# So-bonkers/Detecting-Convolutional-Codes-Via-Markovian-Statistics

Hardware: AMD Instinct MI355X
Metric: MC trials/sec at N=1e5, rate-1/2 m=6 pair, 1/2/4/8 GPUs; Pd match vs CPU (higher is better)
Workload: dtype u32 bit-planes (metrics, four planes of the 64 states) + f64 (log-likelihood sums)

## Files before the change

### detecting-convolutional-codes-via-markovian-statistics_amd/csrc/cvd_device.h

```cpp
#pragma once
#ifndef __HIPCC_RTC__
#include <hip/hip_runtime.h>
#include <stdint.h>
#include <stddef.h>
#else
typedef unsigned char uint8_t;
typedef int int32_t;
typedef unsigned int uint32_t;
typedef long long int64_t;
typedef unsigned long long uint64_t;
typedef __SIZE_TYPE__ size_t;
#endif
#include "cvd_keys.h"
#include "cvd_bitslice.h"

namespace cvd_dev {

using cvd::kEmptyKey;
using cvd::row_words_c;
using cvd::key_hash;

constexpr int kBlock = 256;
#ifndef CVD_K1B_LDSF
#define CVD_K1B_LDSF 0
// ... 60 lines not shown
  if ((threadIdx.x & 63) == 0) {
    if (b1) atomicAdd(reinterpret_cast<unsigned long long*>(counts), (unsigned long long)__popcll(b1));
    if (b2) atomicAdd(reinterpret_cast<unsigned long long*>(counts + 1), (unsigned long long)__popcll(b2));
  }
}

__device__ __forceinline__ int early_decide(double lp, double lr, int64_t rem, double lt_min, double lp_min) {
  const double f = 1.0 + (double)(4 * rem + 32) * 0x1p-53;
  if (lp <= (lr + (double)rem * lt_min) * f) return 1;
  if ((lp + (double)rem * lp_min) * f > lr) return 2;
  return 0;
}
__device__ __forceinline__ void early_final(int dec, double& lp, double& lr) {
  if (dec == 1) { lp = -1.0; lr = 0.0; }
  if (dec == 2) { lp = 1.0; lr = 0.0; }
}
constexpr int kEarlyEvery = 128;


struct ExpArgs {
  const uint32_t* filt;
  const uint32_t* hkey;
  const uint32_t* hrow;
  const uint32_t* drow;
  const uint32_t* dkey;
  const uint32_t* t2;
  const double* ltref;
  const uint32_t* bmp;
  uint32_t repmap, swmap;
  uint32_t bfly_uni;
  uint32_t bfly_even[4];
  uint32_t hmask, fmask, fmask4;
  uint32_t ksh, rsh;
  int32_t max_probe;
  int32_t slot0;
  double lp_unseen;
  int64_t N, nseq, n_h1;
  const uint32_t* r;
  double* sums;
  int64_t* counts;
  uint8_t* trace;
  int32_t early;
  int32_t walk;
  int32_t walk_wmin, walk_amin, walk_burst;
  double lt_min, lp_min;
  int32_t* err;
  const uint32_t* pf;
  uint32_t* wq;
  int32_t mix;
  int32_t t2c;
  int32_t nvtab;
  uint32_t vtab_off;
  const double* vtab;
  int32_t ck_n;
  int32_t ck_len, ck_warm;
  uint32_t* ck_out;
};
constexpr int kCkRecWords = 20;

template <int n>
struct StreamReader {
  static constexpr int SPW = 32 / n;
  static constexpr uint32_t MASK = (1u << n) - 1u;
  const uint32_t* r;
  int64_t pitch, q, N, nwords, wi;
  uint4 cache;
// ... 781 lines not shown
```

### detecting-convolutional-codes-via-markovian-statistics_amd/csrc/cvd_host.cpp

```cpp
#include <atomic>
#include <chrono>
#include <functional>
#include <map>
#include <mutex>
#include <thread>
#include <tuple>
#include <cstdlib>
#include <exception>
#include <cstdio>
#include <algorithm>
#include <cmath>
#include <cstring>
#include <memory>
#include <new>
#include <stdexcept>
#include <string>
#include <unordered_map>
#include <vector>

#include <sys/stat.h>
#include <unistd.h>

#include "../../include/cvd.h"
#include "cvd_internal.h"
// ... 486 lines not shown
    Mo.h_key_slot[(size_t)i] = (uint32_t)slot;
    slot_of[(size_t)i] = (int64_t)slot;
  }
  pt.mark("  nibble tables: hash + insert");
  Mo.h_dkey.assign((size_t)Mo.n_rows * nw, 0u);
  const Tabs T = make_tabs(Mo.dec);
  parallel_for(Mo.n_rows, [&](int64_t i, int) {
    uint32_t* dw = Mo.h_drow.data() + (size_t)dev_of[(size_t)i] * Mo.h_rsw;
    const uint8_t* D = Mo.keys.data() + (size_t)i * M;
    uint8_t succ[16][256];
    for (int r = 0; r < R; ++r) step_host(T, D, (uint32_t)r, succ[r]);
    for (int r = 0; r < R; ++r) {
      std::memcpy(dw + 4 * r, Mo.logp1.data() + (size_t)i * R + r, sizeof(double));
      const int64_t j = Mo.row_next[(size_t)i * R + r];
      dw[4 * r + 2] = (uint32_t)(j >= 0 ? (int32_t)dev_of[(size_t)j] : -1);
      uint32_t c = 0u;
      for (int q2 = 0; q2 < R; ++q2) c += std::memcmp(succ[q2], succ[r], (size_t)M) == 0;
      dw[4 * r + 3] = c;
    }
    std::memcpy(Mo.h_dkey.data() + (size_t)dev_of[(size_t)i] * nw, kws.data() + (size_t)i * nw,
                sizeof(uint32_t) * (size_t)nw);
    uint32_t* hw = interleave ? Mo.h_key_rows.data() + (size_t)i * ssw + nw
                              : Mo.h_row_rows.data() + (size_t)i * Mo.h_rsw;
    std::memcpy(hw, dw, sizeof(uint32_t) * Mo.h_rsw);
  });
  Mo.slot0 = (int32_t)dev_of[0];
  pt.mark("  nibble tables: records");
  Mo.bs = bitslice_preferred(Mo);
  int bload = 3;
  if (const char* e = std::getenv("CVD_BS_LOAD_LOG2")) bload = std::max(1, std::min(5, std::atoi(e)));
  int64_t bcap = 64;
  while (bcap < ((int64_t)1 << bload) * Mo.n_rows) bcap <<= 1;
  constexpr int kSlotW = 64;
  if (bcap * 4 * kSlotW > ((int64_t)1 << 32) || Mo.n_rows * 512 > ((int64_t)1 << 32)) Mo.bs = false;
  Mo.h_bfilt.clear(); Mo.h_bfilt_lds.clear(); Mo.h_bkey_rows.clear(); Mo.h_bkey_slot.clear(); Mo.h_bdkey.clear();
  Mo.h_bpf.clear();
  Mo.bhcap = 0; Mo.bmax_probe = 0;
  if (Mo.bs) {
    Mo.bs_pat_bits = kFilterPatBits;
    if (const char* e = std::getenv("CVD_BS_PAT_BITS")) Mo.bs_pat_bits = std::max(8, std::min(kFilterPatBits, std::atoi(e)));
    const bool bpf = bs_pf_preferred(Mo, ldsf);
    if (bpf) {
      Mo.bs_pat_bits = std::min(Mo.bs_pat_bits, (int32_t)kFilterPatBitsLds);
      Mo.bs_pf_log2 = kBsPfLog2Bits;
      if (const char* e = std::getenv("CVD_BS_PF_LOG2")) Mo.bs_pf_log2 = std::max(16, std::min(20, std::atoi(e)));
      Mo.h_bpf.assign((size_t)1 << (Mo.bs_pf_log2 - 5), 0u);
    }
    const unsigned bnpat = 1u << Mo.bs_pat_bits;
    Mo.bhcap = bcap;
    constexpr int kRecW = 48, kImgW = 48;
    Mo.h_bkey_rows.assign((size_t)Mo.n_rows * kSlotW, 0u);
    Mo.h_bkey_slot.assign((size_t)Mo.n_rows, 0u);
    Mo.h_bfilt.assign((size_t)fcap, 0u);
    Mo.h_bfilt_lds.assign(ldsf ? (size_t)fcap : 0u, 0u);
    Mo.h_bdkey.assign((size_t)Mo.n_rows * kImgW, 0u);
    pt.mark("  bit-sliced tables: allocate");
    std::vector<uint32_t> bph((size_t)Mo.n_rows), bpl((size_t)Mo.n_rows);
    parallel_for(Mo.n_rows, [&](int64_t i, int) {
      uint32_t z[2];
      bs_digest(Mo.keys.data() + (size_t)i * M, z);
      bs_key_hash(z[0], z[1], bph[(size_t)i], bpl[(size_t)i]);
    });
    std::vector<uint8_t> used((size_t)bcap, 0);
    for (int64_t i = 0; i < Mo.n_rows; ++i) {
      const uint32_t ph = bph[(size_t)i], pl = bpl[(size_t)i];
      const size_t fb = (size_t)filter_block_index(pl, (uint32_t)(fcap / 2 - 1));
      Mo.h_bfilt[2 * fb] |= filter_pattern(filter_pattern_index(ph, bnpat));
// ... 632 lines not shown
```

### detecting-convolutional-codes-via-markovian-statistics_amd/csrc/cvd_k1s.h

```cpp
#pragma once

#if defined(CVD_K1S_SLOT3) || defined(CVD_K1S_DEEP) || defined(CVD_K1S_T2) || defined(CVD_K1S_TRIM) || \
    defined(CVD_K1S_MIDPOS) || defined(CVD_K1S_VMASK) || defined(CVD_K1S_PADV) || defined(CVD_K1S_ABL) || \
    defined(CVD_WALK_BUF) || defined(CVD_K1S_AMASK) || defined(CVD_K1S_R16) || defined(CVD_K1S_NT_STREAM) || \
    defined(CVD_BS_ETAB2)
#error "removed k1s knob: CVD_K1S_SLOT3, CVD_K1S_DEEP, CVD_K1S_T2, CVD_K1S_TRIM, CVD_K1S_MIDPOS, CVD_K1S_VMASK, CVD_K1S_PADV, CVD_K1S_ABL, CVD_WALK_BUF, CVD_K1S_AMASK, CVD_K1S_R16, CVD_K1S_NT_STREAM and CVD_BS_ETAB2 no longer exist (DESIGN.md §10)"
#endif

#ifndef CVD_K1B_BITSLICE
#define CVD_K1B_BITSLICE 0
#endif

namespace cvd_dev {

constexpr int kBsSlotShift = 6;
constexpr int kBsRecWord = 48;
template <int PH>
__device__ __forceinline__ constexpr uint32_t bs_img_off() { return 32u * PH; }
constexpr uint32_t kBsRecOff = 4u * kBsRecWord;
constexpr int kBsDkeyWords = 48;
constexpr int kBsEarlyGroups = 21;
#ifndef CVD_K1S_PF
#define CVD_K1S_PF 0
#endif
// ... 43 lines not shown
  }
}
template <int PH, bool kUni, class Mid>
__device__ __forceinline__ void bs_core_tab(const uint32_t (&R)[2][4], uint32_t rr, uint32_t (&N)[2][4], uint32_t& c,
                                            bool& one, Mid mid) {
  const uint2 E0 = *reinterpret_cast<const uint2*>(reinterpret_cast<const char*>(bs_e0_lds()) + PH * 64 + rr);
  const uint32_t e0[2] = {E0.x, E0.y};
  uint32_t mu;
  cvd::bs_step_core_tab<PH, kUni>(
      R, e0,
      [&](bool zero_hit) {
        const char* tb = reinterpret_cast<const char*>(bs_mt_lds()) + PH * 128;
        const uint32_t o = rr + (zero_hit ? 0u : 64u);
        const uint4 w0 = *reinterpret_cast<const uint4*>(tb + o);
        const uint4 w1 = *reinterpret_cast<const uint4*>(tb + o + kBsMtSub);
        const uint2 q = *reinterpret_cast<const uint2*>(tb + o + 2u * kBsMtSub);
        cvd::BsMu T;
        T.e0m[0] = w0.x; T.a1[0] = w0.y; T.p1[0] = w0.z; T.a23[0] = w0.w;
        T.e0m[1] = w1.x; T.a1[1] = w1.y; T.p1[1] = w1.z; T.a23[1] = w1.w;
        T.p23[0] = q.x; T.p23[1] = q.y;
        return T;
      },
      N, mu, c, mid, &one);
}
__device__ __forceinline__ void bs_lt_add(double& lr, const double* s_lt, double lt1, uint32_t c, bool one) {
  if (__builtin_expect(one, 1)) {
    lr += lt1;
  } else {
    lr += s_lt[c];
    asm volatile("" : "+v"(lr));
  }
}

struct BsCursor {
  int32_t slot, pnx;
  uint32_t hs, hsn, fb, fw, fb1, fw1, pc;
  bool cand;
  bool pfpos = true;
  bool h2wave = false;
  double plp;
  uint32_t pkey[8];
  uint32_t vhmask = 0u, vfmask4 = 0u;
  uint32_t half;
  __device__ void prefetch_row(const ExpArgs& a, int32_t s, uint32_t rn) {
    uint32_t o;
    asm("v_lshl_add_u32 %0, %1, 6, %2" : "=v"(o) : "v"((uint32_t)s), "v"(rn));
    const uint4 v = ld_off<uint4>(a.drow, o);
    pc = v.w;
    pnx = (int32_t)v.z;
    plp = __hiloint2double((int)v.y, (int)v.x);
  }
  __device__ void start(const ExpArgs& a, uint32_t r0) {
    slot = a.slot0; hs = 0u; hsn = 0u; fb = 0u; fw = 0u; fb1 = 0u; fw1 = 0u; cand = false; pc = 1u; half = 0u;
    prefetch_row(a, slot, r0);
  }
  __device__ void fence_mid(uint32_t dep) {
    asm volatile("" : "+v"(fw), "+v"(fw1), "+v"(slot) : "v"(dep));
  }
  __device__ void fence_resolve(uint32_t dep) {
    asm volatile("" : "+v"(slot), "+v"(pnx), "+v"(plp), "+v"(pc) : "v"(dep));
#pragma unroll
    for (int w = 0; w < 8; ++w) asm volatile("" : "+v"(pkey[w]) : "v"(dep));
  }
  __device__ static uint32_t slot_off(uint32_t s) { return s << (kBsSlotShift + 2); }
  __device__ static void load_image(const uint32_t* base, uint32_t o, uint32_t (&k)[8]) {
    const uint4 u = ld_off<uint4>(base, o), v = ld_off<uint4>(base, o + 16u);
    k[0] = u.x; k[1] = u.y; k[2] = u.z; k[3] = u.w; k[4] = v.x; k[5] = v.y; k[6] = v.z; k[7] = v.w;
  }
  template <int PH>
  __device__ void mid(const ExpArgs& a, uint32_t r) {
    cand = slot == -2 && cvd::bs_bop3<cvd::kTtAndNotOr>(fb1, fw1, cvd::bs_bop3<cvd::kTtAndNotOr>(fb, fw, 0u)) == 0u;
    if (cand) {
      const uint32_t so = slot_off(hs);
      load_image(a.hkey, so + bs_img_off<PH>(), pkey);
      const uint4 v = ld_off<uint4>(a.hkey, so + kBsRecOff + r);
      pc = v.w;
      pnx = (int32_t)v.z;
      plp = __hiloint2double((int)v.y, (int)v.x);
    }
  }
  __device__ static bool same(const uint32_t (&k)[8], const uint32_t (&R)[2][4]) {
    uint32_t d = k[0] ^ R[0][0];
    d = cvd::bs_bop3<cvd::kTtXorOr>(k[1], R[0][1], d);
    d = cvd::bs_bop3<cvd::kTtXorOr>(k[2], R[0][2], d);
    d = cvd::bs_bop3<cvd::kTtXorOr>(k[3], R[0][3], d);
    d = cvd::bs_bop3<cvd::kTtXorOr>(k[4], R[1][0], d);
    d = cvd::bs_bop3<cvd::kTtXorOr>(k[5], R[1][1], d);
    d = cvd::bs_bop3<cvd::kTtXorOr>(k[6], R[1][2], d);
    d = cvd::bs_bop3<cvd::kTtXorOr>(k[7], R[1][3], d);
    asm volatile("" : "+v"(d));
    return d == 0u;
  }
  template <int PH>
  __device__ double resolve(const ExpArgs& a, const uint32_t (&R)[2][4], uint32_t r, double lpu) {
    const uint32_t m = (uint32_t)(slot >> 31);
    double lpv = lpu;
    int32_t ns = -2;
    ns = (int32_t)cvd::bs_bop3<cvd::kTtSel>(m, (uint32_t)-2, (uint32_t)pnx);
    lpv =
        __hiloint2double((int)cvd::bs_bop3<cvd::kTtSel>(m, (uint32_t)__double2hiint(lpu), (uint32_t)__double2hiint(plp)),
                         (int)cvd::bs_bop3<cvd::kTtSel>(m, (uint32_t)__double2loint(lpu), (uint32_t)__double2loint(plp)));
    if (cand) {
      if (same(pkey, R)) {
        lpv = plp; ns = pnx;
      } else if (pc != 0u) {
        uint32_t sl = hs;
        for (int pr = 1; pr <= a.max_probe; ++pr) {
          sl = (sl + 1u) & a.hmask;
          const uint32_t so = slot_off(sl);
          const uint4 v = ld_off<uint4>(a.hkey, so + kBsRecOff + r);
          if (v.w == 0u) break;
          uint32_t k[8];
          load_image(a.hkey, so + bs_img_off<PH>(), k);
          if (same(k, R)) {
            lpv = __hiloint2double((int)v.y, (int)v.x);
            ns = (int32_t)v.z;
            break;
          }
        }
      }
    }
    slot = ns;
    half = 0u;
    return lpv;
  }
  template <int PH>
  __device__ void hash_ahead(const ExpArgs& a, const uint32_t (&N)[2][4]) {
    uint32_t ph, pl;
    cvd::bs_digest_hash<PH>(N, ph, pl);
    hsn = ph & a.hmask;
    const uint2 pp = *reinterpret_cast<const uint2*>(reinterpret_cast<const char*>(filter_patterns_lds()) +
                                                     (ph & (uint32_t)((cvd::kFilterPatterns - 1) << 3)));
    fb = pp.x;
    fb1 = pp.y;
#if CVD_K1S_PF
    const uint32_t pfw = reinterpret_cast<const uint32_t*>(dyn_lds())[__builtin_amdgcn_ubfe(
        pl, 32 - cvd::kBsPfLog2Bits + 5, cvd::kBsPfLog2Bits - 5)];
    const uint32_t pbit = __builtin_amdgcn_ubfe(pfw, pl >> (32 - cvd::kBsPfLog2Bits), 1u);
    const uint32_t pm = 0u - pbit, sm = (uint32_t)(slot >> 31);
    fb = cvd::bs_bop3<0xF3>(fb, pm, 0u);
    fb1 = cvd::bs_bop3<0xF3>(fb1, pm, 0u);
    const uint32_t fo = cvd::bs_bop3<0x80>(pl, pm, sm) & a.fmask4;
#else
    const uint32_t fo = slot < 0 ? (pl & a.fmask4) : 0u;
#endif
#if CVD_K1B_LDSF
    const uint2 f = *reinterpret_cast<const uint2*>(reinterpret_cast<const char*>(dyn_lds()) + fo);
#else
    const uint2 f = ld_off<uint2>(a.filt, fo);
#endif
    fw = f.x;
    fw1 = f.y;
  }
  template <bool kRow = true>
  __device__ void next(const ExpArgs& a, uint32_t rn) {
    if (kRow && slot >= 0) prefetch_row(a, slot, rn);
    hs = hsn;
  }
};

template <int PH, bool kUni>
__device__ __forceinline__ void bs_step(const ExpArgs& a, BsCursor& cur, const uint32_t (&R)[2][4], uint32_t rr,
                                        uint32_t (&N)[2][4], uint32_t& c, bool& one) {
  bs_core_tab<PH, kUni>(R, rr, N, c, one, [&](uint32_t dep) {
    cur.fence_mid(dep);
    cur.template mid<PH>(a, rr);
  });
  cur.template hash_ahead<(PH + 1) % 6>(a, N);
  cur.fence_resolve(N[1][3]);
}

template <uint64_t XM>
__device__ __forceinline__ void k1s_walk(const ExpArgs& a, int64_t qwave, uint64_t vmask, const double* s_lt) {
  constexpr bool kUni = xm_uni<6, XM>();
  if (CVD_WALK_ABL & 1) return;
  const bool valid = qwave + lane_id() < a.nseq;
  const uint32_t N = (uint32_t)a.N;
  const uint32_t nwords = (N + 15u) / 16u;
  const size_t cstride = (size_t)a.nseq * 4;
  auto load_word = [&](uint32_t wi) -> uint32_t {
    if (wi >= nwords) return 0u;
    return a.r[(size_t)(wi >> 2) * cstride + (size_t)(qwave + lane_id()) * 4 + (wi & 3u)];
  };
  uint32_t pos = 0u, curw = 0u, nxtw = 0u;
  bool need = false;
  auto cur_word = [&]() -> uint32_t { return curw; };
  auto nxt_word = [&]() -> uint32_t { return nxtw; };
  auto word_at = [&]() -> uint32_t { return cur_word() >> (2u * (pos & 15u)); };
  auto advance = [&]() {
    ++pos;
    if ((pos & 15u) == 0u) {
      curw = nxtw;
      need = true;
    }
  };
  uint32_t R[2][4] = {{0u, 0u, 0u, 0u}, {0u, 0u, 0u, 0u}};
  double lp = 0.0, lr = 0.0;
  BsCursor cur;
  cur.slot = -1; cur.pnx = -1; cur.hs = 0u; cur.hsn = 0u; cur.fb = 0u; cur.fw = 0u; cur.fb1 = 0u; cur.fw1 = 0u;
// ... 15 lines not shown
      uint32_t o;
      asm("v_lshl_add_u32 %0, %1, 5, %2" : "=v"(o) : "v"(x & 15u), "v"((uint32_t)cur.slot << 9));
      const uint4 v = ld_off<uint4>(a.t2, o);
      const uint2 w = ld_off<uint2>(a.t2, o + 16u);
      cur.pc = w.y;
      cur.pnx = (int32_t)w.x;
      plp2 = __hiloint2double((int)v.w, (int)v.z);
      cur.plp = __hiloint2double((int)v.y, (int)v.x);
    } else {
      cur.prefetch_row(a, cur.slot, word_param(x & 3u));
    }
  };
  uint32_t mode = kWalkDone;
  int dec = 0;
  auto finished = [&]() -> bool {
    if (pos == N) return true;
    if (a.early && (pos & (uint32_t)(kEarlyEvery - 1)) == 0u) dec = early_decide(lp, lr, (int64_t)(N - pos), a.lt_min, a.lp_min);
    return dec != 0;
  };
  if (valid && N > 0u) {
    curw = load_word(0u);
    nxtw = load_word(1u);
    cur.slot = a.slot0;
    walk_prefetch();
    mode = kWalkWalk;
  }
  uint32_t phw = 0u;
  const double lt1 = a.ltref[1];
  auto acs_step = [&](auto phc) {
    constexpr int PH = decltype(phc)::value;
    const uint32_t rr = word_param(word_at() & 3u);
    uint32_t Nn[2][4], c;
    bool one;
    bs_step<PH, kUni>(a, cur, R, rr, Nn, c, one);
    if (mode == kWalkAcs) {
      lp += cur.template resolve<PH>(a, R, rr, a.lp_unseen);
      bs_lt_add(lr, s_lt, lt1, c, one);
      advance();
      cur.template next<false>(a, 0u);
      if (finished()) {
        mode = kWalkDone;
        cur.slot = -1;
      } else if (cur.slot >= 0) {
        mode = kWalkWalk;
        walk_prefetch();
      }
    }
#pragma unroll
    for (int r = 0; r < 2; ++r)
#pragma unroll
      for (int i = 0; i < 4; ++i) R[r][i] = Nn[r][i];
  };
  const uint32_t wmin = (uint32_t)a.walk_wmin, amin = (uint32_t)a.walk_amin;
  const int burst = a.walk_burst;
  for (int64_t it = 0, it_max = CVD_WALK_GUARD * ((int64_t)N + 1); it < it_max; ++it) {
    if (need) {
      nxtw = load_word((pos >> 4) + 1u);
      need = false;
    }
    const uint64_t mA = __ballot(mode == kWalkAcs), mW = __ballot(mode == kWalkWalk);
    if ((mA | mW) == 0u) break;
    const uint32_t nA = (uint32_t)__popcll(mA), nW = (uint32_t)__popcll(mW);
    if (nW != 0u && (nA == 0u || nW >= wmin || nA < amin)) {
      for (int b = 0; b < burst; ++b) {
        if (mode == kWalkWalk) {
          auto leave = [&]() {
            if (CVD_WALK_ABL & 8) {
              cur.slot = a.slot0;
              advance();
              if (finished()) {
                mode = kWalkDone;
                cur.slot = -1;
// ... 104 lines not shown
  }
  if ((CVD_WALK_ABL & 4) && a.walk) return;
  double lp = 0.0, lr = 0.0;
  if (valid) {
    uint32_t R[2][4] = {{0u, 0u, 0u, 0u}, {0u, 0u, 0u, 0u}};
    double lpu = a.lp_unseen;
    asm volatile("" : "+v"(lpu));
    const int64_t N = a.N, nwords = (N + 15) / 16;
    const size_t cstride = (size_t)a.nseq * 4;
    constexpr bool ck = kCk;
    int64_t t_begin = 0, t_sum = 0, t_end = N;
    if (ck) {
      t_sum = (int64_t)ck_j * a.ck_len;
      t_end = min(N, t_sum + (int64_t)a.ck_len);
      t_begin = max((int64_t)0, t_sum - (int64_t)a.ck_warm);
    }
    uint32_t c4[4];
    auto load_chunk = [&](int64_t ci) {
      const uint32_t* rb = a.r + (size_t)ci * cstride + (size_t)qwave * 4;
      const uint4 v = 4 * ci < nwords ? stream_load(reinterpret_cast<const uint4*>(rb + lane_id() * 4u))
                                      : make_uint4(0u, 0u, 0u, 0u);
      c4[0] = v.x; c4[1] = v.y; c4[2] = v.z; c4[3] = v.w;
    };
    auto pick = [&](int64_t wi) -> uint32_t {
      const uint32_t e = (uint32_t)wi & 3u;
      const uint32_t v = e == 0u ? c4[0] : e == 1u ? c4[1] : e == 2u ? c4[2] : c4[3];
      return wi < nwords ? v : 0u;
    };
    int64_t wi = t_begin / 16;
    load_chunk(wi >> 2);
    uint32_t cw = pick(wi), nw = pick(wi + 1);
    uint32_t sh = 0u;
    BsCursor cur;
    cur.start(a, word_param(cw & 3u));
    const double lt1 = a.ltref[1];
    auto step = [&](auto phc, uint32_t rr, uint32_t rn) {
      constexpr int PH = decltype(phc)::value;
      uint32_t Nn[2][4], c;
      bool one;
      bs_step<PH, kUni>(a, cur, R, rr, Nn, c, one);
      lp += cur.template resolve<PH>(a, R, rr, lpu);
      bs_lt_add(lr, s_lt, lt1, c, one);
#pragma unroll
      for (int r = 0; r < 2; ++r)
#pragma unroll
        for (int i = 0; i < 4; ++i) R[r][i] = Nn[r][i];
      cur.next(a, rn);
    };
    int64_t t = t_begin;
    int grp = 0, dec = 0;
    auto wk = [&](uint32_t w5, auto kc) -> uint32_t {
      constexpr uint32_t k = decltype(kc)::value;
      return (w5 >> (k + 1)) & 0x30u;
    };
    for (; t + 6 <= t_end; t += 6) {
      if (ck && t == t_sum) {
        ck_store(a, qwave, ck_j, 0u, R);
        lp = 0.0;
        lr = 0.0;
      }
      const uint32_t win = __builtin_amdgcn_alignbit(nw, cw, sh);
      const uint32_t w5 = win << 5;
      step(IntC<0>{}, wk(w5, IntC<0>{}), wk(w5, IntC<2>{}));
      step(IntC<1>{}, wk(w5, IntC<2>{}), wk(w5, IntC<4>{}));
      step(IntC<2>{}, wk(w5, IntC<4>{}), wk(w5, IntC<6>{}));
      step(IntC<3>{}, wk(w5, IntC<6>{}), wk(w5, IntC<8>{}));
      step(IntC<4>{}, wk(w5, IntC<8>{}), wk(w5, IntC<10>{}));
      step(IntC<5>{}, wk(w5, IntC<10>{}), wk(w5, IntC<12>{}));
      sh += 12u;
      if (sh >= 32u) {
        sh -= 32u;
        ++wi;
        cw = nw;
        nw = pick(wi + 1);
        if (((wi + 1) & 3) == 3) load_chunk((wi + 2) >> 2);
      }
      if (a.early && ++grp == kBsEarlyGroups) {
        grp = 0;
        if (!dec) dec = early_decide(lp, lr, N - (t + 6), a.lt_min, a.lp_min);
        if (__ballot(dec == 0) == 0) {
          t = N;
          break;
        }
      }
    }
    const int ntail = (int)(t_end - t);
    (void)ntail;
    if (t < t_end) {
      if (ck && t == t_sum) {
        ck_store(a, qwave, ck_j, 0u, R);
        lp = 0.0;
        lr = 0.0;
      }
      const uint32_t win = __builtin_amdgcn_alignbit(nw, cw, sh);
      const uint32_t w5 = win << 5;
      step(IntC<0>{}, wk(w5, IntC<0>{}), wk(w5, IntC<2>{}));
      if (t + 1 < t_end) step(IntC<1>{}, wk(w5, IntC<2>{}), wk(w5, IntC<4>{}));
      if (t + 2 < t_end) step(IntC<2>{}, wk(w5, IntC<4>{}), wk(w5, IntC<6>{}));
      if (t + 3 < t_end) step(IntC<3>{}, wk(w5, IntC<6>{}), wk(w5, IntC<8>{}));
      if (t + 4 < t_end) step(IntC<4>{}, wk(w5, IntC<8>{}), wk(w5, IntC<10>{}));
    }
    if (ck) {
      ck_store(a, qwave, ck_j, 8u, R);
      uint32_t l = lane_id();
      asm volatile("" : "+v"(l));
      double* ps = reinterpret_cast<double*>(
          a.ck_out + ((size_t)ck_j * (size_t)a.nseq + (size_t)qwave + l) * kCkRecWords + 16u);
      ps[0] = lp;
      ps[1] = lr;
      return;
    }
    if (a.sums) {
      const int64_t qe = qwave + lane_id();
      a.sums[2 * qe] = lp;
      a.sums[2 * qe + 1] = lr;
    }
    early_final(dec, lp, lr);
  }
  if constexpr (kCk) return;
  count_decisions_masked(vmask, hmask, lp, lr, a.counts);
// ... 66 lines not shown
```

### detecting-convolutional-codes-via-markovian-statistics_amd/csrc/cvd_kernels.hip

```cpp
#include <hip/hip_runtime.h>

#include <algorithm>
#include <atomic>
#include <cstdlib>
#include <cstring>
#include <map>
#include <mutex>
#include <string>

#include "../../include/cvd.h"
#include "cvd_common.h"
#include "cvd_internal.h"
#include "cvd_device.h"

using namespace cvd;

#define HIP_CHECK(x)                                                                      \
  do {                                                                                    \
    hipError_t e_ = (x);                                                                  \
    if (e_ != hipSuccess) {                                                               \
      set_error(std::string("HIP error '") + hipGetErrorString(e_) + "' at " #x);          \
      return CVD_E_HIP;                                                                   \
    }                                                                                     \
  } while (0)
// ... 1240 lines not shown
}

ExpKernel pick_explicit(int m, int k, int n) {
  if (k == 1 && n == 2) {
    switch (m) {
      case 2: return detect_explicit_kernel<2, 1, 2>;
      case 3: return detect_explicit_kernel<3, 1, 2>;
      case 4: return detect_explicit_kernel<4, 1, 2>;
      case 5: return detect_explicit_kernel<5, 1, 2>;
      case 6: return detect_explicit_kernel<6, 1, 2>;
    }
  }
  if (m == 4 && k == 2 && n == 3) return detect_explicit_kernel<4, 2, 3>;
  return nullptr;
}

template <typename T>
int dev_copy(T*& d, const std::vector<T>& h) {
  if (h.empty()) return CVD_OK;
  HIP_CHECK(hipMalloc(&d, h.size() * sizeof(T)));
  HIP_CHECK(hipMemcpy(d, h.data(), h.size() * sizeof(T), hipMemcpyHostToDevice));
  return CVD_OK;
}

__global__ __launch_bounds__(kBlock) void dir_scatter_kernel(const uint32_t* rows, const uint32_t* slots, int64_t n,
                                                             int32_t w, uint32_t* dir) {
  const int64_t idx = (int64_t)blockIdx.x * kBlock + threadIdx.x;
  if (idx >= n * w) return;
  const int64_t i = idx / w, k = idx - i * w;
  dir[(size_t)slots[i] * (size_t)w + (size_t)k] = rows[idx];
}

int dev_directory(uint32_t*& d, const std::vector<uint32_t>& rows, const std::vector<uint32_t>& slots, int64_t cap,
                  int32_t w, uint32_t fill) {
  if (rows.empty() || cap <= 0) return CVD_OK;
  const int64_t n = (int64_t)slots.size();
  if ((int64_t)rows.size() != n * w) { set_error("directory rows / slots mismatch"); return CVD_E_INVALID; }
  HIP_CHECK(hipMalloc(&d, (size_t)cap * (size_t)w * sizeof(uint32_t)));
  HIP_CHECK(hipMemsetD32(d, (int)fill, (size_t)cap * (size_t)w));
  uint32_t *dr = nullptr, *ds = nullptr;
  HIP_CHECK(hipMalloc(&dr, rows.size() * sizeof(uint32_t)));
  HIP_CHECK(hipMalloc(&ds, slots.size() * sizeof(uint32_t)));
  HIP_CHECK(hipMemcpy(dr, rows.data(), rows.size() * sizeof(uint32_t), hipMemcpyHostToDevice));
  HIP_CHECK(hipMemcpy(ds, slots.data(), slots.size() * sizeof(uint32_t), hipMemcpyHostToDevice));
  const unsigned grid = (unsigned)((n * w + kBlock - 1) / kBlock);
  hipLaunchKernelGGL(dir_scatter_kernel, dim3(grid), dim3(kBlock), 0, 0, dr, ds, n, w, d);
  HIP_CHECK(hipGetLastError());
  HIP_CHECK(hipDeviceSynchronize());
  HIP_CHECK(hipFree(dr));
  HIP_CHECK(hipFree(ds));
  return CVD_OK;
}

}


int cvd::check_device(const cvd_model& M) {
  if (M.device < 0) { set_error("model not uploaded (cvd_model_upload)"); return CVD_E_STATE; }
  int cur = -1;
  HIP_CHECK(hipGetDevice(&cur));
  if (cur != M.device) { set_error("current device differs from the model's device"); return CVD_E_INVALID; }
  return CVD_OK;
}

namespace {
GenArgs gen_args(const CodeDesc& enc, uint32_t k0, uint32_t k1, uint32_t tag, uint64_t thr, int64_t N,
                 int random_input) {
  GenArgs a;
  a.enc = enc; a.k0 = k0; a.k1 = k1; a.tag = tag;
  a.thr_all = thr >= (1ull << 32); a.thr_lo = (uint32_t)std::min<uint64_t>(thr, 0xFFFFFFFFull);
  a.random_input = random_input; a.N = N;
  a.seq_base = 0; a.seq_stride = 1; a.pitch = 0; a.q0 = 0; a.count = 0; a.r = nullptr;
// ... 299 lines not shown
  const bool bs = M.rtc_fn ? M.rtc_bs : bitslice_preferred(M);
  return walk_preferred(M) || (env_i("CVD_LDSF_LOCKSTEP", bs ? 1 : 0) == 1);
}
bool cvd::ldsf_preferred(const cvd_model& M) {
  return !std::getenv("CVD_NO_LDSF") && ldsf_wanted(M) && M.n_rows <= ldsf_max_rows(M.bs) &&
         M.fcap <= ((int64_t)1 << ldsf_log2(M.bs)) && M.h_filt_lds.size() == (size_t)M.fcap;
}

bool cvd::walk_preferred(const cvd_model& M, bool early) {
  const int e = env_i("CVD_WALK", -1);
  if (e >= 0) return e != 0;
  if (M.rtc_fn ? M.rtc_bs : bitslice_preferred(M)) return false;
  return !early && M.kind == 1 && M.learn_len_eff > 0 && 10 * M.n_rows < M.learn_len_eff;
}

static int64_t persist_cap(const cvd_model& M) {
  if (!M.rtc_fn || !M.rtc_bs || M.rtc_persist_grid <= 0 || env_i("CVD_K1S_PERSIST", 1) == 0) return 0;
  int64_t g = M.rtc_persist_grid;
  if (const int pb = env_i("CVD_K1S_PERSIST_BLOCKS", 0); pb > 0) g = std::min<int64_t>(g, pb);
  return g;
}
int64_t cvd::persist_seqs(const cvd_model& M) { return persist_cap(M) * M.rtc_block; }
int64_t cvd::persist_grid(const cvd_model& M, int64_t nseq) {
  const int64_t g = persist_cap(M);
  return g > 0 && (nseq + M.rtc_block - 1) / M.rtc_block > g ? g : 0;
}

static unsigned rtc_dyn_lds(const cvd_model& M) {
  if (M.rtc_ldsf) return (unsigned)(M.fcap * sizeof(uint32_t) + (M.rtc_t2c ? M.h_vtab.size() * sizeof(double) : 0));
  if (M.rtc_pf) return (unsigned)(M.h_bpf.size() * sizeof(uint32_t));
  return 0u;
}

static ExpArgs exp_args(const cvd_model& M, int which, const uint32_t* d_r, int64_t N, int64_t nseq, int64_t n_h1,
                        double* d_sums, int64_t* d_counts, uint8_t* d_trace, const uint32_t* bmp, bool early) {
  ExpArgs a;
  const bool bs = which == CVD_KERNEL_BUTTERFLY_RTC && M.rtc_bs;
  a.filt = which == CVD_KERNEL_BUTTERFLY_RTC && M.rtc_ldsf ? (bs ? M.d_bfilt_lds : M.d_filt_lds)
                                                            : (bs ? M.d_bfilt : M.d_filt);
  a.hkey = bs ? M.d_bkey : M.d_hkey; a.drow = M.d_drow; a.ltref = M.d_ltref;
  a.hrow = bs ? M.d_bkey : M.d_hrow ? M.d_hrow : M.d_hkey + nib_words(M.dec.m);
  a.ksh = bs ? 8u : (uint32_t)__builtin_ctz((unsigned)(4 * M.h_ssw));
  a.rsh = bs ? 8u : M.d_hrow ? (uint32_t)__builtin_ctz((unsigned)(4 * M.h_rsw)) : a.ksh;
  a.bmp = bmp; a.slot0 = M.slot0;
  a.repmap = M.repmap; a.swmap = M.swmap; a.bfly_uni = M.bfly_uni;
  for (int w = 0; w < 4; ++w) a.bfly_even[w] = M.bfly_even[w];
  a.hmask = (uint32_t)((bs ? M.bhcap : M.hcap) - 1); a.fmask = (uint32_t)(M.fcap / 2 - 1); a.fmask4 = a.fmask << 3;
  a.max_probe = bs ? M.bmax_probe : M.max_probe; a.lp_unseen = M.logp1_unseen;
  a.N = N; a.nseq = nseq; a.n_h1 = n_h1; a.r = d_r; a.sums = d_sums; a.counts = d_counts;
  a.trace = d_trace;
  a.early = early && !d_sums && !d_trace; a.lt_min = M.ltref[1]; a.lp_min = M.lp_min;
  a.dkey = bs ? M.d_bdkey : M.d_dkey;
  a.err = M.d_err;
  a.pf = bs && M.rtc_pf ? M.d_bpf : nullptr;
  a.wq = nullptr;
  a.ck_n = 0; a.ck_len = 0; a.ck_warm = 0; a.ck_out = nullptr;
  {
    const int e = env_i("CVD_K1S_MIX", -1);
    a.mix = e >= 0 ? (e != 0) : (M.kind == 1 && M.learn_len_eff > 0 && 2 * M.n_rows < M.learn_len_eff);
  }
  a.t2 = (!M.h_t2.empty() && !std::getenv("CVD_WALK_NOT2")) ? M.d_t2 : nullptr;
  a.t2c = 0; a.nvtab = 0; a.vtab_off = 0u; a.vtab = nullptr;
  if (a.t2 && which == CVD_KERNEL_BUTTERFLY_RTC && M.rtc_bs && M.rtc_ldsf && M.rtc_t2c) {
    a.t2 = M.d_t2c;
    a.t2c = 1;
    a.vtab = M.d_vtab;
    a.nvtab = (int32_t)M.h_vtab.size();
    a.vtab_off = (uint32_t)(M.fcap * sizeof(uint32_t));
  }
  a.walk = which == CVD_KERNEL_BUTTERFLY_RTC && !d_trace && N < ((int64_t)1 << 31) && M.d_dkey && walk_preferred(M, a.early);
  a.walk_wmin = env_i("CVD_WALK_WMIN", 48);
  a.walk_amin = env_i("CVD_WALK_AMIN", 4);
  a.walk_burst = a.t2 ? std::max(1, std::min(7, env_i("CVD_WALK_BURST", 7)))
                      : std::max(1, std::min(16, env_i("CVD_WALK_BURST", 16)));
// ... 249 lines not shown
    for (int32_t c : v) tot += c;
  cvd::ck_last[3] = tot;
  return rc;
}

std::string cvd::rtc_variant_defs(int block, bool ldsf, int patbits, bool bs, bool pf, int pf_log2) {
  return "-DCVD_K1B_BLOCK=" + std::to_string(block) + (ldsf ? " -DCVD_K1B_LDSF=1" : "") +
         (patbits != kFilterPatBits ? " -DCVD_FILTER_PAT_BITS=" + std::to_string(patbits) : "") +
         (bs ? " -DCVD_K1B_BITSLICE=1" : "") + (pf ? " -DCVD_K1S_PF=1" : "") +
         (pf && pf_log2 != kBsPfLog2Bits ? " -DCVD_K1S_PF_LOG2=" + std::to_string(pf_log2) : "");
}

int cvd::upload_model(cvd_model& M, int device) {
  if (M.device == device) return CVD_OK;
  if (M.device >= 0) free_model_device(M);
  int cur = 0;
  HIP_CHECK(hipGetDevice(&cur));
  struct Restore {
    int d;
    ~Restore() { (void)hipSetDevice(d); }
  } restore{cur};
  HIP_CHECK(hipSetDevice(device));
  int rc;
  if ((rc = dev_copy(M.d_ltref, M.ltref))) return rc;
  if (M.kind == 0) {
    if ((rc = dev_copy(M.d_rec, M.rec))) return rc;
    if ((rc = dev_copy(M.d_logp1, M.logp1))) return rc;
  }
  if (M.hcap > 0) {
    if ((rc = dev_copy(M.d_filt, M.h_filt))) return rc;
    if ((rc = dev_copy(M.d_filt_lds, M.h_filt_lds))) return rc;
    if ((rc = dev_directory(M.d_hkey, M.h_key_rows, M.h_key_slot, M.hcap, M.h_ssw, kEmptyKey))) return rc;
    if ((rc = dev_directory(M.d_hrow, M.h_row_rows, M.h_key_slot, M.hcap, M.h_rsw, 0u))) return rc;
    if ((rc = dev_copy(M.d_drow, M.h_drow))) return rc;
    if ((rc = dev_copy(M.d_dkey, M.h_dkey))) return rc;
    if ((rc = dev_copy(M.d_t2, M.h_t2))) return rc;
    if ((rc = dev_copy(M.d_t2c, M.h_t2c))) return rc;
    if ((rc = dev_copy(M.d_vtab, M.h_vtab))) return rc;
    if ((rc = dev_copy(M.d_bfilt, M.h_bfilt))) return rc;
    if ((rc = dev_copy(M.d_bfilt_lds, M.h_bfilt_lds))) return rc;
    if ((rc = dev_directory(M.d_bkey, M.h_bkey_rows, M.h_bkey_slot, M.bhcap, 1 << cvd_dev::kBsSlotShift, 0u))) return rc;
    if ((rc = dev_copy(M.d_bdkey, M.h_bdkey))) return rc;
    if ((rc = dev_copy(M.d_bpf, M.h_bpf))) return rc;
    if ((rc = dev_copy(M.d_bmp, M.bmp))) return rc;
    if ((rc = dev_copy(M.d_bmk1, M.bmk1))) return rc;
    if ((rc = dev_copy(M.d_bfly, M.bfly))) return rc;
  }
  HIP_CHECK(hipMalloc((void**)&M.d_err, sizeof(int32_t)));
  HIP_CHECK(hipMemset(M.d_err, 0, sizeof(int32_t)));
  M.device = device;
  M.lp_min = M.kind == 1 ? M.logp1_unseen : 0.0;
  for (double v : M.logp1) M.lp_min = std::min(M.lp_min, v);
  M.rtc_fn = nullptr;
  M.rtc_fn_multi = nullptr;
  M.rtc_fn_walk = nullptr;
  M.rtc_fn_multi_walk = nullptr;
  M.rtc_nowalk = false;
  M.jit_error.clear();
  M.rtc_ldsf = M.k1b_ok && M.hcap > 0 && ldsf_preferred(M);
  M.rtc_bs = false;
  M.rtc_pf = false;
  for (int attempt = M.bs && M.d_bkey ? 0 : 1; attempt < 2 && M.k1b_ok && M.hcap > 0; ++attempt) {
    const bool bs = attempt == 0;
    const bool pf = bs && !M.rtc_ldsf && M.d_bpf != nullptr;
    M.rtc_block = pf ? (M.bs_pf_log2 >= 20 ? 1024 : 512) : env_i("CVD_K1B_BLOCK", M.rtc_ldsf ? (M.fcap > ((int64_t)1 << 14) ? 1024 : 512) : kBlock);
    if (M.rtc_block != 256 && M.rtc_block != 512 && M.rtc_block != 1024) M.rtc_block = kBlock;
    const int patbits = M.rtc_ldsf ? kFilterPatBitsLds : bs ? M.bs_pat_bits : kFilterPatBits;
    const std::string wdefs = rtc_variant_defs(M.rtc_block, M.rtc_ldsf, patbits, bs, pf, M.bs_pf_log2);
    const bool nowalk = bs && !walk_preferred(M) && env_i("CVD_K1S_WALK_CODE", 0) == 0;
    const std::string vdefs = wdefs + (nowalk ? kNoWalkDef : "");
    if (rtc_k1b_function(device, M.dec.m, M.bfly_x, vdefs.c_str(), &M.rtc_fn, &M.rtc_fn_multi) == 0) {
      M.rtc_bs = bs;
      M.rtc_pf = pf;
      M.rtc_nowalk = nowalk;
// ... 4 lines not shown
    M.rtc_fn = nullptr;
    M.rtc_fn_multi = nullptr;
    M.jit_error = last_error_copy();
  }
  if (!M.rtc_fn) {
    M.rtc_ldsf = false;
    M.rtc_block = kBlock;
  }
  M.rtc_t2c = false;
  if (M.rtc_fn && M.rtc_bs && M.rtc_ldsf && M.d_t2c && M.d_vtab) {
    int st = 0, mx = 0;
    if (hipFuncGetAttribute(&st, HIP_FUNC_ATTRIBUTE_SHARED_SIZE_BYTES, (hipFunction_t)M.rtc_fn) == hipSuccess &&
        hipDeviceGetAttribute(&mx, hipDeviceAttributeMaxSharedMemoryPerMultiprocessor, device) == hipSuccess &&
        (int64_t)st + M.fcap * 4 + (int64_t)M.h_vtab.size() * 8 <= (int64_t)mx)
      M.rtc_t2c = true;
  }
  M.rtc_persist_grid = 0;
  if (M.rtc_fn && M.rtc_bs) {
    int nb = 0, ncu = 0;
    if (hipModuleOccupancyMaxActiveBlocksPerMultiprocessor(&nb, (hipFunction_t)M.rtc_fn, M.rtc_block,
                                                           rtc_dyn_lds(M)) == hipSuccess &&
        hipDeviceGetAttribute(&ncu, hipDeviceAttributeMultiprocessorCount, device) == hipSuccess && nb > 0 && ncu > 0) {
      M.rtc_persist_grid = (int64_t)nb * ncu;
    }
  }
  return CVD_OK;
}

void cvd::free_model_device(cvd_model& M) {
  if (M.device < 0) return;
  int cur = 0;
  (void)hipGetDevice(&cur);
  (void)hipSetDevice(M.device);
  void* ptrs[] = {M.d_rec, M.d_logp1, M.d_ltref, M.d_filt, M.d_filt_lds, M.d_hkey, M.d_hrow, M.d_drow, M.d_dkey, M.d_t2,
                  M.d_t2c, M.d_vtab, M.d_bmp,
                  M.d_bmk1, M.d_bfly, M.d_err, M.d_bfilt, M.d_bfilt_lds, M.d_bkey, M.d_bdkey, M.d_bpf};
  for (void* p : ptrs)
    if (p) (void)hipFree(p);
  M.d_rec = nullptr; M.d_logp1 = nullptr; M.d_ltref = nullptr;
  M.d_filt = nullptr; M.d_filt_lds = nullptr; M.d_hkey = nullptr; M.d_hrow = nullptr; M.d_drow = nullptr; M.d_dkey = nullptr; M.d_t2 = nullptr;
  M.d_t2c = nullptr; M.d_vtab = nullptr; M.rtc_t2c = false;
  M.d_bfilt = nullptr; M.d_bfilt_lds = nullptr; M.d_bkey = nullptr; M.d_bdkey = nullptr; M.d_bpf = nullptr;
  M.rtc_persist_grid = 0;
  M.rtc_bs = false;
  M.rtc_pf = false;
  M.rtc_nowalk = false;
  M.rtc_fn_walk = nullptr;
  M.rtc_fn_multi_walk = nullptr;
  M.d_bmp = nullptr;
  M.d_bmk1 = nullptr;
  M.d_bfly = nullptr;
  M.d_err = nullptr;
  M.rtc_fn = nullptr;
  M.rtc_fn_multi = nullptr;
  M.device = -1;
  (void)hipSetDevice(cur);
}


namespace {
int parse_code_dev(const cvd_code* c, CodeDesc& d) {
  if (!c || !c->taps || c->k < 1 || c->k > kMaxK || c->n < 1 || c->n > kMaxN || c->m < 1 || c->m > kMaxM) {
    set_error("bad code description");
    return CVD_E_INVALID;
  }
  d.k = c->k; d.n = c->n; d.m = c->m;
// ... 397 lines not shown
```

Measured before the change: 1.520 million.

## Merge dense row table into bitslice key buffer for single per-step row load

Appends the dense row table (drow) to the end of the bitslice key directory allocation so both live in one buffer addressed from the same base. The per-step row fetch is moved into mid(), where one conditional 16-byte load picks either the candidate slot's record or the dense row depending on the hash state. This replaces the separate prefetch in next() plus the record load on candidates. The goal is fewer outstanding global loads per trellis step and fewer registers held across the step. In exchange, a wave-uniform ballot is added, the load sits later in the step (less prefetch distance), and the 32-bit offset limit check now has to include the appended table.

Measured after the change: 1.546 million, median of 6. +1.7%, better.

```diff
diff --git a/detecting-convolutional-codes-via-markovian-statistics_amd/csrc/cvd_device.h b/detecting-convolutional-codes-via-markovian-statistics_amd/csrc/cvd_device.h
--- a/detecting-convolutional-codes-via-markovian-statistics_amd/csrc/cvd_device.h
+++ b/detecting-convolutional-codes-via-markovian-statistics_amd/csrc/cvd_device.h
@@ -116,6 +116,7 @@
   uint32_t bfly_even[4];
   uint32_t hmask, fmask, fmask4;
   uint32_t ksh, rsh;
+  uint32_t rec_off;
   int32_t max_probe;
   int32_t slot0;
   double lp_unseen;
diff --git a/detecting-convolutional-codes-via-markovian-statistics_amd/csrc/cvd_host.cpp b/detecting-convolutional-codes-via-markovian-statistics_amd/csrc/cvd_host.cpp
--- a/detecting-convolutional-codes-via-markovian-statistics_amd/csrc/cvd_host.cpp
+++ b/detecting-convolutional-codes-via-markovian-statistics_amd/csrc/cvd_host.cpp
@@ -542,7 +542,7 @@
   int64_t bcap = 64;
   while (bcap < ((int64_t)1 << bload) * Mo.n_rows) bcap <<= 1;
   constexpr int kSlotW = 64;
-  if (bcap * 4 * kSlotW > ((int64_t)1 << 32) || Mo.n_rows * 512 > ((int64_t)1 << 32)) Mo.bs = false;
+  if (bcap * 4 * kSlotW + Mo.n_rows * 4 * (int64_t)Mo.h_rsw > ((int64_t)1 << 32) || Mo.n_rows * 512 > ((int64_t)1 << 32)) Mo.bs = false;
   Mo.h_bfilt.clear(); Mo.h_bfilt_lds.clear(); Mo.h_bkey_rows.clear(); Mo.h_bkey_slot.clear(); Mo.h_bdkey.clear();
   Mo.h_bpf.clear();
   Mo.bhcap = 0; Mo.bmax_probe = 0;
diff --git a/detecting-convolutional-codes-via-markovian-statistics_amd/csrc/cvd_k1s.h b/detecting-convolutional-codes-via-markovian-statistics_amd/csrc/cvd_k1s.h
--- a/detecting-convolutional-codes-via-markovian-statistics_amd/csrc/cvd_k1s.h
+++ b/detecting-convolutional-codes-via-markovian-statistics_amd/csrc/cvd_k1s.h
@@ -99,27 +99,29 @@
   }
 }
 
+#if CVD_K1B_LDSF
+constexpr bool kBsOneLoad = false;
+#else
+constexpr bool kBsOneLoad = true;
+#endif
 struct BsCursor {
   int32_t slot, pnx;
   uint32_t hs, hsn, fb, fw, fb1, fw1, pc;
   bool cand;
-  bool pfpos = true;
-  bool h2wave = false;
   double plp;
   uint32_t pkey[8];
-  uint32_t vhmask = 0u, vfmask4 = 0u;
-  uint32_t half;
   __device__ void prefetch_row(const ExpArgs& a, int32_t s, uint32_t rn) {
     uint32_t o;
     asm("v_lshl_add_u32 %0, %1, 6, %2" : "=v"(o) : "v"((uint32_t)s), "v"(rn));
-    const uint4 v = ld_off<uint4>(a.drow, o);
+    take(ld_off<uint4>(a.drow, o));
+  }
+  __device__ void take(const uint4& v) {
     pc = v.w;
     pnx = (int32_t)v.z;
     plp = __hiloint2double((int)v.y, (int)v.x);
   }
-  __device__ void start(const ExpArgs& a, uint32_t r0) {
-    slot = a.slot0; hs = 0u; hsn = 0u; fb = 0u; fw = 0u; fb1 = 0u; fw1 = 0u; cand = false; pc = 1u; half = 0u;
-    prefetch_row(a, slot, r0);
+  __device__ void start(const ExpArgs& a) {
+    slot = a.slot0; pnx = -1; hs = 0u; hsn = 0u; fb = 0u; fw = 0u; fb1 = 0u; fw1 = 0u; cand = false; pc = 1u; plp = 0.0;
   }
   __device__ void fence_mid(uint32_t dep) {
     asm volatile("" : "+v"(fw), "+v"(fw1), "+v"(slot) : "v"(dep));
@@ -134,16 +136,27 @@
     const uint4 u = ld_off<uint4>(base, o), v = ld_off<uint4>(base, o + 16u);
     k[0] = u.x; k[1] = u.y; k[2] = u.z; k[3] = u.w; k[4] = v.x; k[5] = v.y; k[6] = v.z; k[7] = v.w;
   }
-  template <int PH>
+  template <int PH, bool kRow>
   __device__ void mid(const ExpArgs& a, uint32_t r) {
     cand = slot == -2 && cvd::bs_bop3<cvd::kTtAndNotOr>(fb1, fw1, cvd::bs_bop3<cvd::kTtAndNotOr>(fb, fw, 0u)) == 0u;
-    if (cand) {
+    if constexpr (kRow && kBsOneLoad) {
+      bs_u32x4 v;
+      if (__ballot(cand || slot >= 0) != 0u) {
+        static_assert(kBsRecOff == 192u && kBsSlotShift == 6, "a slot's records are its fourth 64-B unit");
+        uint32_t uc, o;
+        asm("v_lshl_or_b32 %0, %1, 2, 3" : "=v"(uc) : "v"(hs));
+        const uint32_t ud = (uint32_t)slot + (a.rec_off >> 6);
+        asm("v_lshl_add_u32 %0, %1, 6, %2" : "=v"(o) : "v"(cand ? uc : ud), "v"(r));
+        v = ld_off<bs_u32x4>(a.hkey, o);
+      } else {
+        asm volatile("" : "=v"(v));
+      }
+      take(make_uint4(v.x, v.y, v.z, v.w));
+      if (cand) load_image(a.hkey, slot_off(hs) + bs_img_off<PH>(), pkey);
+    } else if (cand) {
       const uint32_t so = slot_off(hs);
       load_image(a.hkey, so + bs_img_off<PH>(), pkey);
-      const uint4 v = ld_off<uint4>(a.hkey, so + kBsRecOff + r);
-      pc = v.w;
-      pnx = (int32_t)v.z;
-      plp = __hiloint2double((int)v.y, (int)v.x);
+      take(ld_off<uint4>(a.hkey, so + kBsRecOff + r));
     }
   }
   __device__ static bool same(const uint32_t (&k)[8], const uint32_t (&R)[2][4]) {
@@ -161,10 +174,8 @@
   template <int PH>
   __device__ double resolve(const ExpArgs& a, const uint32_t (&R)[2][4], uint32_t r, double lpu) {
     const uint32_t m = (uint32_t)(slot >> 31);
-    double lpv = lpu;
-    int32_t ns = -2;
-    ns = (int32_t)cvd::bs_bop3<cvd::kTtSel>(m, (uint32_t)-2, (uint32_t)pnx);
-    lpv =
+    int32_t ns = (int32_t)cvd::bs_bop3<cvd::kTtSel>(m, (uint32_t)-2, (uint32_t)pnx);
+    double lpv =
         __hiloint2double((int)cvd::bs_bop3<cvd::kTtSel>(m, (uint32_t)__double2hiint(lpu), (uint32_t)__double2hiint(plp)),
                          (int)cvd::bs_bop3<cvd::kTtSel>(m, (uint32_t)__double2loint(lpu), (uint32_t)__double2loint(plp)));
     if (cand) {
@@ -188,7 +199,6 @@
       }
     }
     slot = ns;
-    half = 0u;
     return lpv;
   }
   template <int PH>
@@ -219,19 +229,19 @@
     fw = f.x;
     fw1 = f.y;
   }
-  template <bool kRow = true>
-  __device__ void next(const ExpArgs& a, uint32_t rn) {
-    if (kRow && slot >= 0) prefetch_row(a, slot, rn);
-    hs = hsn;
+  __device__ void next() { hs = hsn; }
+  __device__ void next_row(const ExpArgs& a, uint32_t rn) {
+    if (slot >= 0) prefetch_row(a, slot, rn);
+    next();
   }
 };
 
-template <int PH, bool kUni>
+template <int PH, bool kUni, bool kRow = true>
 __device__ __forceinline__ void bs_step(const ExpArgs& a, BsCursor& cur, const uint32_t (&R)[2][4], uint32_t rr,
                                         uint32_t (&N)[2][4], uint32_t& c, bool& one) {
   bs_core_tab<PH, kUni>(R, rr, N, c, one, [&](uint32_t dep) {
     cur.fence_mid(dep);
-    cur.template mid<PH>(a, rr);
+    cur.template mid<PH, kRow>(a, rr);
   });
   cur.template hash_ahead<(PH + 1) % 6>(a, N);
   cur.fence_resolve(N[1][3]);
@@ -313,12 +323,12 @@
     const uint32_t rr = word_param(word_at() & 3u);
     uint32_t Nn[2][4], c;
     bool one;
-    bs_step<PH, kUni>(a, cur, R, rr, Nn, c, one);
+    bs_step<PH, kUni, false>(a, cur, R, rr, Nn, c, one);
     if (mode == kWalkAcs) {
       lp += cur.template resolve<PH>(a, R, rr, a.lp_unseen);
       bs_lt_add(lr, s_lt, lt1, c, one);
       advance();
-      cur.template next<false>(a, 0u);
+      cur.next();
       if (finished()) {
         mode = kWalkDone;
         cur.slot = -1;
@@ -489,7 +499,8 @@
     uint32_t cw = pick(wi), nw = pick(wi + 1);
     uint32_t sh = 0u;
     BsCursor cur;
-    cur.start(a, word_param(cw & 3u));
+    cur.start(a);
+    if constexpr (!kBsOneLoad) cur.prefetch_row(a, cur.slot, word_param(cw & 3u));
     const double lt1 = a.ltref[1];
     auto step = [&](auto phc, uint32_t rr, uint32_t rn) {
       constexpr int PH = decltype(phc)::value;
@@ -502,7 +513,8 @@
       for (int r = 0; r < 2; ++r)
 #pragma unroll
         for (int i = 0; i < 4; ++i) R[r][i] = Nn[r][i];
-      cur.next(a, rn);
+      if constexpr (kBsOneLoad) cur.next();
+      else cur.next_row(a, rn);
     };
     int64_t t = t_begin;
     int grp = 0, dec = 0;
@@ -541,8 +553,6 @@
         }
       }
     }
-    const int ntail = (int)(t_end - t);
-    (void)ntail;
     if (t < t_end) {
       if (ck && t == t_sum) {
         ck_store(a, qwave, ck_j, 0u, R);
diff --git a/detecting-convolutional-codes-via-markovian-statistics_amd/csrc/cvd_kernels.hip b/detecting-convolutional-codes-via-markovian-statistics_amd/csrc/cvd_kernels.hip
--- a/detecting-convolutional-codes-via-markovian-statistics_amd/csrc/cvd_kernels.hip
+++ b/detecting-convolutional-codes-via-markovian-statistics_amd/csrc/cvd_kernels.hip
@@ -1296,12 +1296,14 @@
 }
 
 int dev_directory(uint32_t*& d, const std::vector<uint32_t>& rows, const std::vector<uint32_t>& slots, int64_t cap,
-                  int32_t w, uint32_t fill) {
+                  int32_t w, uint32_t fill, const std::vector<uint32_t>* tail = nullptr) {
   if (rows.empty() || cap <= 0) return CVD_OK;
   const int64_t n = (int64_t)slots.size();
   if ((int64_t)rows.size() != n * w) { set_error("directory rows / slots mismatch"); return CVD_E_INVALID; }
-  HIP_CHECK(hipMalloc(&d, (size_t)cap * (size_t)w * sizeof(uint32_t)));
+  const size_t ntail = tail ? tail->size() : 0u;
+  HIP_CHECK(hipMalloc(&d, ((size_t)cap * (size_t)w + ntail) * sizeof(uint32_t)));
   HIP_CHECK(hipMemsetD32(d, (int)fill, (size_t)cap * (size_t)w));
+  if (ntail) HIP_CHECK(hipMemcpy(d + (size_t)cap * (size_t)w, tail->data(), ntail * sizeof(uint32_t), hipMemcpyHostToDevice));
   uint32_t *dr = nullptr, *ds = nullptr;
   HIP_CHECK(hipMalloc(&dr, rows.size() * sizeof(uint32_t)));
   HIP_CHECK(hipMalloc(&ds, slots.size() * sizeof(uint32_t)));
@@ -1667,6 +1669,8 @@
   return 0u;
 }
 
+static size_t bs_rec_words(const cvd_model& M) { return (size_t)M.bhcap << cvd_dev::kBsSlotShift; }
+
 static ExpArgs exp_args(const cvd_model& M, int which, const uint32_t* d_r, int64_t N, int64_t nseq, int64_t n_h1,
                         double* d_sums, int64_t* d_counts, uint8_t* d_trace, const uint32_t* bmp, bool early) {
   ExpArgs a;
@@ -1675,6 +1679,7 @@
                                                             : (bs ? M.d_bfilt : M.d_filt);
   a.hkey = bs ? M.d_bkey : M.d_hkey; a.drow = M.d_drow; a.ltref = M.d_ltref;
   a.hrow = bs ? M.d_bkey : M.d_hrow ? M.d_hrow : M.d_hkey + nib_words(M.dec.m);
+  a.rec_off = bs ? (uint32_t)(bs_rec_words(M) * sizeof(uint32_t)) : 0u;
   a.ksh = bs ? 8u : (uint32_t)__builtin_ctz((unsigned)(4 * M.h_ssw));
   a.rsh = bs ? 8u : M.d_hrow ? (uint32_t)__builtin_ctz((unsigned)(4 * M.h_rsw)) : a.ksh;
   a.bmp = bmp; a.slot0 = M.slot0;
@@ -1990,14 +1995,15 @@
     if ((rc = dev_copy(M.d_filt_lds, M.h_filt_lds))) return rc;
     if ((rc = dev_directory(M.d_hkey, M.h_key_rows, M.h_key_slot, M.hcap, M.h_ssw, kEmptyKey))) return rc;
     if ((rc = dev_directory(M.d_hrow, M.h_row_rows, M.h_key_slot, M.hcap, M.h_rsw, 0u))) return rc;
-    if ((rc = dev_copy(M.d_drow, M.h_drow))) return rc;
     if ((rc = dev_copy(M.d_dkey, M.h_dkey))) return rc;
     if ((rc = dev_copy(M.d_t2, M.h_t2))) return rc;
     if ((rc = dev_copy(M.d_t2c, M.h_t2c))) return rc;
     if ((rc = dev_copy(M.d_vtab, M.h_vtab))) return rc;
     if ((rc = dev_copy(M.d_bfilt, M.h_bfilt))) return rc;
     if ((rc = dev_copy(M.d_bfilt_lds, M.h_bfilt_lds))) return rc;
-    if ((rc = dev_directory(M.d_bkey, M.h_bkey_rows, M.h_bkey_slot, M.bhcap, 1 << cvd_dev::kBsSlotShift, 0u))) return rc;
+    if ((rc = dev_directory(M.d_bkey, M.h_bkey_rows, M.h_bkey_slot, M.bhcap, 1 << cvd_dev::kBsSlotShift, 0u, &M.h_drow))) return rc;
+    if (M.d_bkey) M.d_drow = M.d_bkey + bs_rec_words(M);
+    else if ((rc = dev_copy(M.d_drow, M.h_drow))) return rc;
     if ((rc = dev_copy(M.d_bdkey, M.h_bdkey))) return rc;
     if ((rc = dev_copy(M.d_bpf, M.h_bpf))) return rc;
     if ((rc = dev_copy(M.d_bmp, M.bmp))) return rc;
@@ -2068,6 +2074,7 @@
   int cur = 0;
   (void)hipGetDevice(&cur);
   (void)hipSetDevice(M.device);
+  if (M.d_bkey) M.d_drow = nullptr;
   void* ptrs[] = {M.d_rec, M.d_logp1, M.d_ltref, M.d_filt, M.d_filt_lds, M.d_hkey, M.d_hrow, M.d_drow, M.d_dkey, M.d_t2,
                   M.d_t2c, M.d_vtab, M.d_bmp,
                   M.d_bmk1, M.d_bfly, M.d_err, M.d_bfilt, M.d_bfilt_lds, M.d_bkey, M.d_bdkey, M.d_bpf};
```
